# soon-yau/upgpt

Hardware: AMD Instinct MI355X
Metric: 256x256 images/sec, 50-step DDIM, bs=8/GPU; UNet MFMA util % (higher is better)
Workload: dtype f16; 1 GPU; BASELINE configs[1]: bs=8/GPU, 256x256 px (latent 4x32x32), 50-step DDIM eta=0, text-only cond [B,87,768], UNet(bbox.yaml) + VAE decode, EMA weights, no CFG; batch_per_gpu=8, ddim_steps=50, batches_in_flight_per_gpu=4, lane_hw_queues=measured, parallelism=replica-dp1, one all-gather of images per batch

## Files before the change

### include/upk.h

```cpp
#ifndef UPK_H_
#define UPK_H_

#include <stddef.h>
#include <stdint.h>

#ifdef __cplusplus
extern "C" {
#endif

#define UPK_VERSION 100

#define UPK_OK 0
#define UPK_EINVAL (-1)
#define UPK_ESHAPE (-2)
#define UPK_EWORKSPACE (-3)
#define UPK_EHIP (-4)
#define UPK_ENODEV (-5)

typedef struct upk_ctx upk_ctx;
typedef void* upk_stream;

int upk_version(void);
int upk_create(upk_ctx** out, int device);
int upk_destroy(upk_ctx* ctx);
const char* upk_last_error(upk_ctx* ctx);
int upk_set_workspace(upk_ctx* ctx, void* dptr, size_t bytes);
int upk_num_cus(upk_ctx* ctx);

int upk_pack_weight_f16(upk_ctx* ctx, const float* w_oihw, int cout, int cin, int kh, int kw,
                        const int32_t* row_map, int n_rows_packed, const int32_t* col_map,
                        int cin_packed, void* w_packed, upk_stream stream);
size_t upk_packed_weight_bytes(int n_rows_packed, int cin_packed, int kh, int kw);

#define UPK_F_SILU 0x1
#define UPK_F_GEGLU 0x2
#define UPK_F_OUT_F32 0x4
#define UPK_F_OUT_NCHW_F32 0x8
#define UPK_F_UPSAMPLE2X 0x10
#define UPK_F_PAD_ASYM 0x20
#define UPK_F_QUICKGELU 0x40

typedef struct upk_conv_desc {
  const void* x1;
  const void* x2;
  int32_t c1, c2;
  int32_t ld1, ld2;
  int32_t batch;
  int32_t in_h, in_w;
  int32_t ksize;
  int32_t stride;
  const void* w_packed;
  int32_t n_out;
  int32_t n_pad;
  const float* bias;
  const void* residual;
  int32_t ld_res;
  const float* rowvec;
  int32_t rv_batch_stride;
  int32_t rv_step_stride;
  const int32_t* step;
  void* y;
  int32_t ldy;
  void* vt;
  int32_t vt_from, vt_heads, vt_dhead, vt_ld, vt_tokens;
  int32_t flags;
  int32_t tune_cfg, tune_splitk;
  const float* ln_colsum;
  float ln_eps;
  int32_t ln_dim;
  float* gn_stats_ws;
  int32_t gn_groups;
  const void* x3;
  const void* x4;
  int32_t c3, c4;
  int32_t ld3, ld4;
  const float* gno_gamma;
  const float* gno_beta;
  void* gno_y;
  float gno_eps;
  int32_t gno_silu, gno_ld, gno_skip_y;
  float* ln_rows_out;
  const float* ln_rows_in;
  int32_t ln_rows_slots;
  const void* w_phase;
  int32_t gn_stats_cap;
  const void* pf_next;
  int64_t pf_bytes;
} upk_conv_desc;

int upk_conv2d_nhwc_f16(upk_ctx* ctx, const upk_conv_desc* d, upk_stream stream);

int upk_conv_gn_fused(upk_ctx* ctx, const upk_conv_desc* d, int* mode, int* nblk);
int upk_groupnorm_finalize_f32(upk_ctx* ctx, const float* partials, int nblk, int ld, int batch, int hw, int c,
                               int groups, float* ws, upk_stream stream);
int upk_conv_ln_rows(upk_ctx* ctx, const upk_conv_desc* d, int* slots);

typedef struct upk_mlp_desc {
  const void* x;
  int32_t ldx, m, c, inner;
  const void* w1;
  const float* b1;
  const float* u1;
  float ln_eps;
  int32_t ln_dim;
  const void* w2;
  const float* b2;
  int32_t n_out, n_pad;
  const void* residual;
  int32_t ld_res;
  void* y;
  int32_t ldy;
  float* gn_stats_ws;
  int32_t hw, rows_per_wg;
} upk_mlp_desc;
int upk_geglu_mlp_f16(upk_ctx* ctx, const upk_mlp_desc* d, upk_stream stream);
int upk_geglu_mlp_supported(upk_ctx* ctx, const upk_mlp_desc* d);

typedef struct upk_xblock_desc {
  const void* a1;
  int32_t lda, m, c, heads, d;
  const void* t0;
  int32_t ld_t0;
  const void* w_out1;
  const void* w_q;
  const void* w_out2;
  const float* vec;
  float ln_eps;
  int32_t ln_dim;
  const void* k_ctx;
  int32_t ldk, n_kv;
  const void* vt_ctx;
  int32_t vt_ld;
  float scale;
  void* y;
  int32_t ldy;
  int32_t hw, rows_per_wg;
} upk_xblock_desc;
int upk_cross_block_f16(upk_ctx* ctx, const upk_xblock_desc* d, upk_stream stream);
int upk_cross_block_supported(upk_ctx* ctx, const upk_xblock_desc* d);

typedef struct upk_hblock_desc {
  const void* x;
  int32_t ldx, m, c, heads, d;
  const void* w_in;
  const void* w_qkv;
  const float* vec;
  float ln_eps;
  int32_t ln_dim;
  void* t0;
  int32_t ld_t0;
  void* qk;
  int32_t ld_qk;
  void* vt;
  int32_t vt_ld;
  int32_t hw, rows_per_wg;
  const float* gn_part;
  const float* gn_gamma;
  const float* gn_beta;
  int32_t gn_nblk, gn_ld, gn_groups;
  float gn_eps;
} upk_hblock_desc;
int upk_head_block_f16(upk_ctx* ctx, const upk_hblock_desc* d, upk_stream stream);
int upk_head_block_supported(upk_ctx* ctx, const upk_hblock_desc* d);

int upk_gemm_f16(upk_ctx* ctx, const void* a, int lda, int m, int k, const void* w_packed,
                 int n_out, int n_pad, const float* bias, const void* residual, int ld_res,
                 void* y, int ldy, int flags, upk_stream stream);

int upk_conv_autotune(upk_ctx* ctx, const upk_conv_desc* d, upk_stream stream, int reps, int* best_cfg,
                      int* best_splitk, float* best_us, float* default_us);

int upk_conv_override(upk_ctx* ctx, int cfg, int splitk);
int upk_conv_num_configs(void);
const char* upk_conv_config_name(int cfg);

int upk_attention_f16(upk_ctx* ctx, const void* q, int ldq, long long q_batch_stride,
                      const void* k, int ldk, long long k_batch_stride, const void* vt, int vt_ld,
                      void* out, int ldo, long long o_batch_stride, int batch, int heads, int n_q,
                      int n_kv, int d, float scale, upk_stream stream);
// ... 180 lines not shown
```

### upgpt_amd/_lib.py

```python
import contextlib
import ctypes as C
import os
import threading

import torch
from ._check import require

_HERE = os.path.dirname(os.path.abspath(__file__))
LIB_PATH = os.environ.get("UPK_LIB") or os.path.join(_HERE, "libupk.so")

SYMBOLS = [
    "upk_version", "upk_create", "upk_destroy", "upk_last_error", "upk_set_workspace", "upk_num_cus",
    "upk_pack_weight_f16", "upk_packed_weight_bytes", "upk_conv2d_nhwc_f16", "upk_gemm_f16",
    "upk_conv_autotune", "upk_conv_override", "upk_conv_num_configs", "upk_conv_config_name", "upk_conv_gn_fused",
    "upk_conv_ln_rows",
    "upk_geglu_mlp_f16", "upk_geglu_mlp_supported", "upk_cross_block_f16", "upk_cross_block_supported", "upk_head_block_f16", "upk_head_block_supported",
    "upk_attention_f16", "upk_groupnorm_nhwc_f16", "upk_groupnorm_stats_nhwc_f16", "upk_groupnorm_chunks", "upk_groupnorm_apply_nhwc_f16", "upk_groupnorm_finalize_f32", "upk_groupnorm_ws_bytes",
    "upk_layernorm_f16", "upk_timestep_embed_f16",
    "upk_nchw_f32_to_nhwc_f16", "upk_nhwc_f16_to_nchw_f32", "upk_f32_to_f16", "upk_ddim_step_f32",
    "upk_ddim_step_cfg_f32", "upk_ddim_step_edit_f32", "upk_plms_step_f32", "upk_ddpm_step_f32", "upk_attention_causal_f16", "upk_attention_qproj_f16", "upk_embed_tokens_f16",
    "upk_attention_fewkeys_f16", "upk_gelu_f16",
    "upk_patchify_nchw_f32_f16", "upk_vit_assemble_f16", "upk_gather_rows_f16",
    "upk_image_finish_u8", "upk_resize_bilinear_u8", "upk_segm_boxes_u8", "upk_style_crops_u8",
    "upk_cond_bbox_u8", "upk_cond_gather_u8", "upk_cond_smpl_u8", "upk_clip_normalize_u8", "upk_ssim_ws_bytes", "upk_ssim_u8",
    "upk_lpips_input_f16", "upk_relu_pool_nhwc_f16", "upk_lpips_ws_bytes", "upk_lpips_layer_f16",
    "upk_conv2d_rect_f16", "upk_pool3_nhwc_f16", "upk_fid_input_f16", "upk_avgpool_global_f32",
    "upk_q_sample_f32", "upk_p_losses_ws_bytes", "upk_p_losses_f32",
    "upk_advance_step", "upk_step_autoadvance", "upk_kernel_launches", "upk_graph_begin", "upk_graph_end", "upk_graph_launch", "upk_graph_destroy",
    "upk_prof_enable", "upk_prof_collect",
    "upk_stream_create_cumask", "upk_stream_destroy", "upk_probe_placement", "upk_probe_clock",
]

F_SILU, F_GEGLU, F_OUT_F32, F_OUT_NCHW_F32, F_UPSAMPLE2X, F_PAD_ASYM = 0x1, 0x2, 0x4, 0x8, 0x10, 0x20
DDPM_X0, DDPM_CLIP = 0x1, 0x2
LAYOUT_NCHW, LAYOUT_NHWC = 0, 1
STYLE_FILL, STYLE_MASK = 0x1, 0x2
FINISH_SAMPLE, FINISH_INPUT, FINISH_DENORM = 0, 1, 2
F_QUICKGELU = 0x40
POOL_MAX, POOL_AVG = 0, 1
LOSS_L2, LOSS_L1 = 0, 1
NUM_CLASSES = 5
CLASS_NAMES = ["igemm", "attention", "groupnorm", "layernorm", "other"]

E_NAMES = {0: "UPK_OK", -1: "UPK_EINVAL", -2: "UPK_ESHAPE", -3: "UPK_EWORKSPACE", -4: "UPK_EHIP", -5: "UPK_ENODEV"}


class UpkError(RuntimeError):
    def __init__(self, code, msg):
        super().__init__("%s: %s" % (E_NAMES.get(code, str(code)), msg))
        self.code = code


class ConvDesc(C.Structure):
    _fields_ = [
        ("x1", C.c_void_p), ("x2", C.c_void_p),
        ("c1", C.c_int32), ("c2", C.c_int32), ("ld1", C.c_int32), ("ld2", C.c_int32),
        ("batch", C.c_int32), ("in_h", C.c_int32), ("in_w", C.c_int32),
        ("ksize", C.c_int32), ("stride", C.c_int32),
        ("w_packed", C.c_void_p), ("n_out", C.c_int32), ("n_pad", C.c_int32),
        ("bias", C.c_void_p), ("residual", C.c_void_p), ("ld_res", C.c_int32),
        ("rowvec", C.c_void_p), ("rv_batch_stride", C.c_int32), ("rv_step_stride", C.c_int32),
        ("step", C.c_void_p), ("y", C.c_void_p), ("ldy", C.c_int32),
        ("vt", C.c_void_p), ("vt_from", C.c_int32), ("vt_heads", C.c_int32), ("vt_dhead", C.c_int32),
        ("vt_ld", C.c_int32), ("vt_tokens", C.c_int32), ("flags", C.c_int32),
        ("tune_cfg", C.c_int32), ("tune_splitk", C.c_int32),
        ("ln_colsum", C.c_void_p), ("ln_eps", C.c_float), ("ln_dim", C.c_int32),
        ("gn_stats_ws", C.c_void_p), ("gn_groups", C.c_int32),
        ("x3", C.c_void_p), ("x4", C.c_void_p),
        ("c3", C.c_int32), ("c4", C.c_int32), ("ld3", C.c_int32), ("ld4", C.c_int32),
        ("gno_gamma", C.c_void_p), ("gno_beta", C.c_void_p), ("gno_y", C.c_void_p), ("gno_eps", C.c_float),
        ("gno_silu", C.c_int32), ("gno_ld", C.c_int32), ("gno_skip_y", C.c_int32),
        ("ln_rows_out", C.c_void_p), ("ln_rows_in", C.c_void_p), ("ln_rows_slots", C.c_int32),
        ("w_phase", C.c_void_p), ("gn_stats_cap", C.c_int32),
        ("pf_next", C.c_void_p), ("pf_bytes", C.c_int64),
    ]


class MlpDesc(C.Structure):
    _fields_ = [
        ("x", C.c_void_p), ("ldx", C.c_int32), ("m", C.c_int32), ("c", C.c_int32), ("inner", C.c_int32),
        ("w1", C.c_void_p), ("b1", C.c_void_p), ("u1", C.c_void_p), ("ln_eps", C.c_float), ("ln_dim", C.c_int32),
        ("w2", C.c_void_p), ("b2", C.c_void_p), ("n_out", C.c_int32), ("n_pad", C.c_int32),
        ("residual", C.c_void_p), ("ld_res", C.c_int32), ("y", C.c_void_p), ("ldy", C.c_int32),
        ("gn_stats_ws", C.c_void_p), ("hw", C.c_int32), ("rows_per_wg", C.c_int32),
    ]


class XblockDesc(C.Structure):
    _fields_ = [
        ("a1", C.c_void_p), ("lda", C.c_int32), ("m", C.c_int32), ("c", C.c_int32), ("heads", C.c_int32), ("d", C.c_int32),
        ("t0", C.c_void_p), ("ld_t0", C.c_int32),
        ("w_out1", C.c_void_p), ("w_q", C.c_void_p), ("w_out2", C.c_void_p), ("vec", C.c_void_p),
        ("ln_eps", C.c_float), ("ln_dim", C.c_int32),
        ("k_ctx", C.c_void_p), ("ldk", C.c_int32), ("n_kv", C.c_int32),
        ("vt_ctx", C.c_void_p), ("vt_ld", C.c_int32), ("scale", C.c_float),
        ("y", C.c_void_p), ("ldy", C.c_int32), ("hw", C.c_int32), ("rows_per_wg", C.c_int32),
    ]


class HblockDesc(C.Structure):
    _fields_ = [
        ("x", C.c_void_p), ("ldx", C.c_int32), ("m", C.c_int32), ("c", C.c_int32), ("heads", C.c_int32), ("d", C.c_int32),
        ("w_in", C.c_void_p), ("w_qkv", C.c_void_p), ("vec", C.c_void_p), ("ln_eps", C.c_float), ("ln_dim", C.c_int32),
        ("t0", C.c_void_p), ("ld_t0", C.c_int32), ("qk", C.c_void_p), ("ld_qk", C.c_int32),
        ("vt", C.c_void_p), ("vt_ld", C.c_int32), ("hw", C.c_int32), ("rows_per_wg", C.c_int32),
        ("gn_part", C.c_void_p), ("gn_gamma", C.c_void_p), ("gn_beta", C.c_void_p),
        ("gn_nblk", C.c_int32), ("gn_ld", C.c_int32), ("gn_groups", C.c_int32), ("gn_eps", C.c_float),
    ]


_lib = None
_lib_lock = threading.Lock()


def load_library(path=None):
    global _lib
    with _lib_lock:
        if _lib is not None and path is None:
            return _lib
        p = path or LIB_PATH
        if not os.path.exists(p):
            raise RuntimeError(
                "libupk.so not found at %s: build it with `python -m upgpt_amd.build` "
                "(hipcc --offload-arch=gfx950). There is no CPU fallback." % p)
        lib = C.CDLL(p)
        vp, i32, i64, f32 = C.c_void_p, C.c_int, C.c_longlong, C.c_float
        protos = {
            "upk_version": (C.c_int, []),
            "upk_create": (C.c_int, [C.POINTER(vp), i32]),
            "upk_destroy": (C.c_int, [vp]),
            "upk_last_error": (C.c_char_p, [vp]),
            "upk_set_workspace": (C.c_int, [vp, vp, C.c_size_t]),
            "upk_num_cus": (C.c_int, [vp]),
            "upk_pack_weight_f16": (C.c_int, [vp, vp, i32, i32, i32, i32, vp, i32, vp, i32, vp, vp]),
            "upk_packed_weight_bytes": (C.c_size_t, [i32, i32, i32, i32]),
            "upk_conv2d_nhwc_f16": (C.c_int, [vp, C.POINTER(ConvDesc), vp]),
            "upk_gemm_f16": (C.c_int, [vp, vp, i32, i32, i32, vp, i32, i32, vp, vp, i32, vp, i32, i32, vp]),
            "upk_conv_autotune": (C.c_int, [vp, C.POINTER(ConvDesc), vp, i32, C.POINTER(C.c_int), C.POINTER(C.c_int),
                                            C.POINTER(C.c_float), C.POINTER(C.c_float)]),
            "upk_conv_override": (C.c_int, [vp, i32, i32]),
            "upk_conv_num_configs": (C.c_int, []),
            "upk_conv_config_name": (C.c_char_p, [i32]),
            "upk_conv_ln_rows": (C.c_int, [vp, C.POINTER(ConvDesc), C.POINTER(C.c_int)]),
            "upk_geglu_mlp_f16": (C.c_int, [vp, C.POINTER(MlpDesc), vp]),
            "upk_geglu_mlp_supported": (C.c_int, [vp, C.POINTER(MlpDesc)]),
            "upk_cross_block_f16": (C.c_int, [vp, C.POINTER(XblockDesc), vp]),
            "upk_cross_block_supported": (C.c_int, [vp, C.POINTER(XblockDesc)]),
            "upk_head_block_f16": (C.c_int, [vp, C.POINTER(HblockDesc), vp]),
            "upk_head_block_supported": (C.c_int, [vp, C.POINTER(HblockDesc)]),
            "upk_attention_f16": (C.c_int, [vp, vp, i32, i64, vp, i32, i64, vp, i32, vp, i32, i64,
                                            i32, i32, i32, i32, i32, f32, vp]),
            "upk_attention_causal_f16": (C.c_int, [vp, vp, i32, i64, vp, i32, i64, vp, i32, vp, i32, i64,
                                                   i32, i32, i32, i32, f32, vp]),
            "upk_attention_qproj_f16": (C.c_int, [vp, vp, i32, i64, i32, i32, f32, vp, vp, vp, vp, i32, i64, vp, i32, vp,
                                                  i32, i64, i32, i32, i32, i32, i32, f32, vp]),
            "upk_attention_fewkeys_f16": (C.c_int, [vp, vp, i32, i64, vp, i32, i64, vp, i32, i64, vp, i32, i64,
                                                    i32, i32, i32, i32, i32, f32, vp]),
            "upk_gelu_f16": (C.c_int, [vp, vp, i32, i32, i32, vp]),
# ... 464 lines not shown
```

### upgpt_amd/csrc/mlp.hip

```cpp
#include "igemm_common.h"

namespace upkd {
namespace {

constexpr int ML_NW = 8;

struct MlpArgs {
  const f16* x;
  const f16* w1;
  const f16* w2;
  const f16* zero;
  const float* b1;
  const float* u1;
  const float* b2;
  const f16* res;
  f16* y;
  float* gn_cp;
  int ldx, ldr, ldy, M, nch1, n1, n2, n2pad, nh;
  int gn_nblk, gn_hw;
  float ln_inv_dim, ln_eps;
  unsigned long long* dbg;
};
#define ML_PIN(v) asm volatile("" ::"s"(v))

template <int MI, int PF>
__global__ __launch_bounds__(512) void mlp_kernel(const MlpArgs s) {
  constexpr int NW = ML_NW, NI = 2;
  constexpr int BM = MI * 16;
  constexpr int PW = NW * NI * 16;
  extern __shared__ __attribute__((aligned(16))) f16 smem[];
  ML_PIN(s.x); ML_PIN(s.w1); ML_PIN(s.w2); ML_PIN(s.zero); ML_PIN(s.b1); ML_PIN(s.u1); ML_PIN(s.b2); ML_PIN(s.res);
  ML_PIN(s.y); ML_PIN(s.gn_cp); ML_PIN(s.ldx); ML_PIN(s.ldr); ML_PIN(s.ldy); ML_PIN(s.M); ML_PIN(s.nch1); ML_PIN(s.n1);
  ML_PIN(s.n2); ML_PIN(s.n2pad); ML_PIN(s.nh);

  const int tid = threadIdx.x;
  const int lane = tid & 63;
  const int wave = __builtin_amdgcn_readfirstlane(tid >> 6);
  const int lg = lane >> 4, lc = lane & 15;
#ifdef UPK_TIMELINE
  const bool tl = s.dbg && (blockIdx.x == 0 || blockIdx.x == gridDim.x - 1) && (wave == 0 || wave == 4);
  unsigned long long* tlp = s.dbg + (blockIdx.x == 0 ? 0 : 64) + (wave == 0 ? 0 : 32);
#define STAMP(i) do { if (tl && lane == 0 && (i) < 32) tlp[i] = __builtin_readcyclecounter(); } while (0)
#else
#define STAMP(i) do { } while (0)
#endif
  STAMP(0);
  const int m0 = upk_xcd_tile(blockIdx.x, gridDim.x) * BM;
  const int nch1 = s.nch1, nh = s.nh, nch2 = nh + nch1;
  f16* const hT = smem;
  f16* const xT = smem + nh * BM * 32;
  float* const st = (float*)(smem + nch2 * BM * 32);
  float* const bl = st + BM * 2;

  {
    typedef __attribute__((address_space(3))) void* lds_ptr;
    typedef const __attribute__((address_space(1))) void* glb_ptr;
    const int r16 = lane >> 2;
    const int chd = (lane & 3) ^ ((-(lane >> 4)) & 3);
    const f16* zsrc = s.zero + (lane & 3) * 8;
    for (int idx = wave; idx < nch1 * MI; idx += NW) {
      const int kc = idx / MI, rg = idx - kc * MI;
      const int m = m0 + rg * 16 + r16;
      const f16* src = m < s.M ? s.x + (long)m * s.ldx + kc * 32 + chd * 8 : zsrc;
      __builtin_amdgcn_global_load_lds((glb_ptr)src, (lds_ptr)(xT + (kc * BM + rg * 16) * 32), 16, 0, 0);
    }
    const int nkb = s.n1 >> 8;
    for (int idx = wave; idx < 2 * nkb; idx += NW) {
      const float* src = (idx < nkb ? s.b1 + idx * 256 : s.u1 + (idx - nkb) * 256) + lane * 4;
      __builtin_amdgcn_global_load_lds((glb_ptr)src, (lds_ptr)(bl + idx * 256), 16, 0, 0);
    }
  }

  const int col1 = (wave >> 1) * 64 + (wave & 1) * 16;
  const int npass = (s.n1 + PW - 1) / PW;
  const int p1w = min(npass, (s.n1 - col1 + PW - 1) / PW);
  const int col2 = wave * 32;
  const bool act2 = col2 < s.n2pad;
  const unsigned ks1 = (unsigned)s.n1 * 64u, ks2 = (unsigned)s.n2pad * 64u;
  const unsigned loff = (unsigned)(lc * 32 + lg * 8) * 2u;
  unsigned voff1[PF], voff2[PF];
#pragma unroll
  for (int u = 0; u < PF; ++u) voff1[u] = loff + (unsigned)u * ks1, voff2[u] = loff + (unsigned)u * ks2;
  const char* wb1 = (const char*)s.w1;
  const char* wb2 = (const char*)s.w2 + (size_t)col2 * 64;
  auto base1 = [&](int p, int kc) -> const char* {
    return wb1 + (size_t)(((unsigned)kc * (unsigned)s.n1 + (unsigned)(col1 + p * PW)) * 64u);
  };
  f16x8 ring[PF][NI];
// ... 110 lines not shown
    STAMP(5 + 2 * p);
  }
  STAMP(20);
  __syncthreads();
  STAMP(21);

  if (!act2) return;
  f32x4 acc[MI][NI];
#pragma unroll
  for (int i = 0; i < MI; ++i)
#pragma unroll
    for (int j = 0; j < NI; ++j) acc[i][j] = (f32x4){0.f, 0.f, 0.f, 0.f};
#pragma unroll 1
  for (int kc0 = 0; kc0 < nch2; kc0 += PF) {
    const bool dead = kc0 + PF >= nch2;
    const char* sb0 = dead ? wb2 : wb2 + (size_t)((unsigned)(kc0 + PF) * ks2);
    const char* ldsA = hs + la + (unsigned)(kc0 * BM) * 64u;
#pragma unroll
    for (int u = 0; u < PF; ++u) {
      f16x8 fc[MI];
#pragma unroll
      for (int i = 0; i < MI; ++i) fc[i] = *(const f16x8*)(ldsA + (u * BM + i * 16) * 64);
#pragma unroll
      for (int i = 0; i < MI; ++i)
#pragma unroll
        for (int j = 0; j < NI; ++j)
          acc[i][j] = __builtin_amdgcn_mfma_f32_16x16x32_f16(ring[u][j], fc[i], acc[i][j], 0, 0, 0);
      const unsigned vo = dead ? loff : voff2[u];
      ring[u][0] = *(const f16x8*)(sb0 + vo);
      ring[u][1] = *(const f16x8*)(sb0 + (dead ? 0 : 1024) + vo);
      __builtin_amdgcn_sched_barrier(0);
    }
  }
  STAMP(22);
  f32x4 cs[NI], cq[NI];
#pragma unroll
  for (int j = 0; j < NI; ++j) cs[j] = cq[j] = (f32x4){0.f, 0.f, 0.f, 0.f};
#pragma unroll
  for (int i = 0; i < MI; ++i) {
    const int m = m0 + i * 16 + lc;
    const bool ok = m < s.M;
    f16* yrow = s.y + (unsigned)(ok ? m : 0) * (unsigned)s.ldy;
#pragma unroll
    for (int j = 0; j < NI; ++j) {
      const int n = col2 + j * 16 + lg * 4;
      const f32x4 v = acc[i][j] + b2v[j];
      f16x4 o;
#pragma unroll
      for (int k = 0; k < 4; ++k) o[k] = (f16)(v[k] + (float)rr[i][j][k]);
      if (ok && n < s.n2) *(f16x4*)(yrow + n) = o;
#pragma unroll
      for (int k = 0; k < 4; ++k) {
        const float f = ok ? (float)o[k] : 0.f;
        cs[j][k] += f;
        cq[j][k] += f * f;
      }
    }
  }
  if (s.gn_cp) {
    const int b = m0 / s.gn_hw;
    const int blk = (m0 - b * s.gn_hw) / BM;
    float* dst = s.gn_cp + (long)((b * s.gn_nblk + blk) * 2) * s.n2pad;
#pragma unroll
    for (int j = 0; j < NI; ++j) {
      const int n = col2 + j * 16 + lg * 4;
#pragma unroll
      for (int k = 0; k < 4; ++k) {
        cs[j][k] = Epi::row_sum16(cs[j][k]);
        cq[j][k] = Epi::row_sum16(cq[j][k]);
      }
      if (lc == 0 && n < s.n2pad) {
        *(f32x4*)(dst + n) = cs[j];
        *(f32x4*)(dst + s.n2pad + n) = cq[j];
      }
    }
  }
#ifdef UPK_TIMELINE
  asm volatile("s_waitcnt vmcnt(0)" ::: "memory");
  STAMP(23);
#endif
#undef STAMP
}

}
}

using namespace upkd;

extern "C" int upk_geglu_mlp_supported(upk_ctx* ctx, const upk_mlp_desc* d) {
  if (!ctx || !d) return 0;
  if (d->c <= 0 || (d->c & 31) || d->inner != 4 * d->c || (d->inner & 31)) return 0;
  const int nch1 = d->c / 32, nh = d->inner / 32;
  if (nch1 % 7 || (nch1 + nh) % 7) return 0;
  if (d->n_pad > ML_NW * 32 || (d->n_pad & 31)) return 0;
  if ((d->ldx & 7) || (d->ld_res & 3) || (d->ldy & 3) || (d->n_out & 3)) return 0;
  const int bm = d->rows_per_wg > 0 ? d->rows_per_wg : 64;
  if (bm != 32 && bm != 64) return 0;
  if ((2 * d->inner) & 255) return 0;
  if ((size_t)(nch1 + nh) * bm * 64 + (size_t)bm * 8 + (size_t)d->inner * 16 > 160 * 1024) return 0;
  if (d->gn_stats_ws && (d->hw <= 0 || d->hw % bm || d->hw / bm > UPK_GN_MAX_CHUNKS)) return 0;
  return 1;
}

extern "C" int upk_geglu_mlp_f16(upk_ctx* ctx, const upk_mlp_desc* d, upk_stream stream_) {
  if (!ctx || !d) return UPK_EINVAL;
  if (!d->x || !d->w1 || !d->w2 || !d->b1 || !d->u1 || !d->b2 || !d->residual || !d->y)
    return upk_fail(ctx, UPK_EINVAL, "geglu_mlp: null operand");
  if (!upk_geglu_mlp_supported(ctx, d))
    return upk_fail(ctx, UPK_ESHAPE, "geglu_mlp: shape outside the fused kernel's domain (c=%d inner=%d n_pad=%d)", d->c,
                    d->inner, d->n_pad);
  hipStream_t stream = (hipStream_t)stream_;
  MlpArgs s;
  memset(&s, 0, sizeof(s));
  s.x = (const f16*)d->x, s.w1 = (const f16*)d->w1, s.w2 = (const f16*)d->w2, s.zero = (const f16*)ctx->zero_page;
  s.b1 = d->b1, s.u1 = d->u1, s.b2 = d->b2, s.res = (const f16*)d->residual, s.y = (f16*)d->y;
  s.gn_cp = d->gn_stats_ws;
  s.ldx = d->ldx, s.ldr = d->ld_res, s.ldy = d->ldy, s.M = d->m;
  s.nch1 = d->c / 32, s.n1 = 2 * d->inner, s.n2 = d->n_out, s.n2pad = d->n_pad, s.nh = d->inner / 32;
  const int bm = d->rows_per_wg > 0 ? d->rows_per_wg : 64;
  s.gn_hw = d->hw > 0 ? d->hw : 1;
  s.gn_nblk = d->hw > 0 ? d->hw / bm : 1;
  s.ln_inv_dim = 1.0f / (float)(d->ln_dim > 0 ? d->ln_dim : d->c);
  s.ln_eps = d->ln_eps;
#ifdef UPK_TIMELINE
  s.dbg = getenv("UPK_MLP_TL") ? (unsigned long long*)((char*)ctx->ws + ctx->ws_bytes - 4096) : nullptr;
#endif
  const size_t lds = (size_t)(s.nch1 + s.nh) * bm * 64 + (size_t)bm * 8 + (size_t)s.n1 * 8;
  void (*fn)(const MlpArgs) = bm == 32 ? mlp_kernel<2, 7> : mlp_kernel<4, 7>;
  static unsigned long long attr32 = 0, attr64 = 0;
  if (int rc = upk_lds_attr_once(ctx, (const void*)fn, bm == 32 ? &attr32 : &attr64)) return rc;
  upk_prof_scope prof(ctx, UPK_CLS_IGEMM, stream);
  hipLaunchKernelGGL(fn, dim3((s.M + bm - 1) / bm), dim3(512), lds, stream, s);
  return upk_check_launch(ctx, "geglu_mlp");
}
```

### upgpt_amd/emitter.py

```python
import ctypes as C
import os

import torch

from . import _lib as L
from . import knobs as K
from ._check import require
from .packing import PW, Packer, _rup, head_pad
from .tuning import TUNE_CACHE, TUNE_CACHE_LANES


class Act:
    __slots__ = ("t", "B", "H", "W", "C", "gn_src", "ln_src")

    def __init__(self, t, B, H, W, C):
        self.t, self.B, self.H, self.W, self.C = t, B, H, W, C
        self.ln_src = None
        self.gn_src = None

    @property
    def ld(self):
        return self.t.shape[-1]

    @property
# ... 320 lines not shown
            if os.environ.get("UPGPT_GN_2SRC", "1") != "1":
                return None
            for sr in srcs:
                if isinstance(sr, Emitter.GnProvider):
                    continue
                key = self.convs[sr[1]][1]
                e = TUNE_CACHE.get(key) or TUNE_CACHE.get(key[:-3] if key.endswith("_gs") else key + "_gs")
                if e is None or (e[1] != 1 and not self._is_as(int(e[0]))):
                    return None
        armed = []
        for act in acts:
            if isinstance(act.gn_src, Emitter.GnProvider):
                armed.append((act.gn_src, act.gn_src.sws))
                continue
            d = act.gn_src[0]
            if not d.gn_stats_ws:
                ci = act.gn_src[1]
                cap = max(32, (act.H * act.W) // 64)
                sws = self.alloc(self.ctx.gn_stats_floats(act.B, d.n_pad, cap), dtype=torch.float32)
                d.gn_stats_ws, d.gn_groups, d.gn_stats_cap = sws.data_ptr(), 32, cap
                require(self.convs[ci][0] is d, "conv list out of sync with GroupNorm producers", RuntimeError)
                self.convs[ci] = (d, self.convs[ci][1] + "_gs")
                act.gn_src = (d, ci, sws)
            armed.append((d, act.gn_src[2]))
        return armed

    def groupnorm(self, P, x1, gamma, beta, eps, silu, ws, x2=None, sole=False):
        Cc = x1.C + (x2.C if x2 is not None else 0)
        y = Act(self.alloc(x1.M, Cc), x1.B, x1.H, x1.W, Cc)
        fn, h, chk = self.lib.upk_groupnorm_nhwc_f16, self.hctx, self._chk
        a = (x1.t.data_ptr(), x1.C, x1.ld, x2.t.data_ptr() if x2 is not None else None, x2.C if x2 is not None else 0,
             x2.ld if x2 is not None else 0, x1.B, x1.H * x1.W, 32, gamma.data_ptr(), beta.data_ptr(), float(eps),
             int(bool(silu)), y.t.data_ptr(), y.ld)
        armed = self._arm_gn_sources([x1] if x2 is None else [x1, x2])
        if armed is None:
            P.add(lambda s: chk(fn(h, *a, ws.data_ptr(), s)), x1, x2, gamma, beta, y, ws, cls="groupnorm",
                  label="gn M%d C%d silu%d 2pass" % (x1.M, Cc, int(bool(silu))))
        else:
            fused_fn, apply_fn = self.lib.upk_conv_gn_fused, self.lib.upk_groupnorm_apply_nhwc_f16
            fin_fn = self.lib.upk_groupnorm_finalize_f32
            mine = None
            if K.GN_REDUCE_APPLY and x2 is None and not isinstance(armed[0][0], Emitter.GnProvider) and not armed[0][0].gno_y:
                mine = armed[0][0]
                mine.gno_gamma, mine.gno_beta, mine.gno_eps = gamma.data_ptr(), beta.data_ptr(), float(eps)
                mine.gno_silu, mine.gno_y, mine.gno_ld, mine.gno_skip_y = int(bool(silu)), y.t.data_ptr(), y.ld, int(bool(sole))

            def run(s):
                info = []
                for d, sws in armed:
                    if isinstance(d, Emitter.GnProvider):
                        info.append((2, d.nblk, d.ld, sws.data_ptr()))
                        continue
                    mode, nblk = C.c_int(0), C.c_int(0)
                    chk(fused_fn(h, C.byref(d), C.byref(mode), C.byref(nblk)))
                    info.append((mode.value if mode.value != 3 or d is mine else 0, nblk.value, d.n_pad, sws.data_ptr()))
                if len(info) == 1 and info[0][0] == 3:
                    return
                if len(info) == 1 and info[0][0] == 2 and info[0][1] > 32:
                    m, nb, ld, p1 = info[0]
                    chk(fin_fn(h, p1, nb, ld, x1.B, x1.H * x1.W, x1.C, 32, ws.data_ptr(), s))
                    chk(apply_fn(h, *a, ws.data_ptr(), 1, 0, 0, None, 0, 0, s))
                    return
                if len(info) == 1 and info[0][0]:
                    m, nb, ld, p1 = info[0]
                    chk(apply_fn(h, *a, p1, m, nb, ld, None, 0, 0, s))
                elif len(info) == 2 and info[0][0] == 2 and info[1][0] == 2 and max(info[0][1], info[1][1]) <= 32:
                    chk(apply_fn(h, *a, info[0][3], 2, info[0][1], info[0][2], info[1][3], info[1][1], info[1][2], s))
                else:
                    chk(fn(h, *a, ws.data_ptr(), s))

            P.add(run, x1, x2, gamma, beta, y, ws, armed, cls="groupnorm",
                  label="gn M%d C%d silu%d" % (x1.M, Cc, int(bool(silu))))
        P.n_launch += 1
        return y

    def layernorm(self, P, x, gamma, beta, eps=1e-5):
        y = Act(self.alloc(x.M, x.C), x.B, x.H, x.W, x.C)
        fn, h, chk = self.lib.upk_layernorm_f16, self.hctx, self._chk
        a = (x.t.data_ptr(), x.ld, x.M, x.C, gamma.data_ptr(), beta.data_ptr(), float(eps), y.t.data_ptr(), y.ld)
        P.add(lambda s: chk(fn(h, *a, s)), x, gamma, beta, y, cls="layernorm", label="ln M%d C%d" % (x.M, x.C))
        return y

    def mlp_rows(self, M):
        if K.MLP_ROWS in (32, 64):
            return K.MLP_ROWS
        return 64 if M // 64 >= self.ctx.num_cus else 32

    def geglu_mlp(self, P, t2, x_in, pw1, pw2, gn_stats=True):
        if K.MLP_FUSE == "0" or t2.C != t2.ld:
            return None
        M, C_ = t2.M, t2.C
        if (K.MLP_FUSE == "auto" and L.concurrency() > 1 and os.environ.get("UPGPT_LANES_TUNING", "1") == "1"
                and M in TUNE_CACHE_LANES.meta.get("__unfuse_mlp_M__", ())):
            return None
        rows = self.mlp_rows(M)
        d = L.MlpDesc()
        d.x, d.ldx, d.m, d.c, d.inner = t2.t.data_ptr(), t2.ld, M, C_, pw1.n_out
        d.w1, d.b1, d.u1 = pw1.w.data_ptr(), pw1.bias.data_ptr(), pw1.ln_colsum.data_ptr()
        d.ln_eps, d.ln_dim = 1e-5, C_
        d.w2, d.b2, d.n_out, d.n_pad = pw2.w.data_ptr(), pw2.bias.data_ptr(), pw2.n_out, pw2.n_pad
        d.residual, d.ld_res = x_in.t.data_ptr(), x_in.ld
        hw = t2.H * t2.W
        d.hw, d.rows_per_wg = hw, rows
        if not self.lib.upk_geglu_mlp_supported(self.hctx, C.byref(d)):
            return None
        if K.MLP_FUSE == "auto" and (M + rows - 1) // rows < (self.ctx.num_cus * 3) // 4:
            return None
        out = Act(self.alloc(M, pw2.n_out), t2.B, t2.H, t2.W, pw2.n_out)
        d.y, d.ldy = out.t.data_ptr(), out.ld
        sws = None
        if gn_stats and hw % rows == 0 and hw // rows <= 32:
            sws = self.alloc(self.ctx.gn_stats_floats(t2.B, pw2.n_pad), dtype=torch.float32)
            d.gn_stats_ws = sws.data_ptr()
            out.gn_src = Emitter.GnProvider(sws, hw // rows, pw2.n_pad)
        fn, h, chk = self.lib.upk_geglu_mlp_f16, self.hctx, self._chk
        P.add(lambda s: chk(fn(h, C.byref(d), s)), d, t2, x_in, pw1, pw2, out, sws, cls="igemm_k1",
              label="mlp M%d C%d rows%d" % (M, C_, rows))
        P.igemm_flops += 2 * M * (2 * pw1.n_out * C_ + pw2.n_real * (pw1.n_out + C_))
        P.flops[-1] = 2 * M * (2 * pw1.n_out * C_ + pw2.n_real * (pw1.n_out + C_))
        return out

    def row_chain_rows(self, kind, M, default=32):
        forced = (K.HB_ROWS if kind == "hblock" else 0) or K.XB_ROWS
        if forced:
            return forced
        if L.concurrency() > 1 and os.environ.get("UPGPT_LANES_TUNING", "1") == "1":
            r = TUNE_CACHE_LANES.meta.get("__row_chain_rows__", {}).get(kind, {}).get(str(M))
            if r:
                return int(r)
        return default

    def head_block_ok(self, x, t, heads, dp, qk, vt_ld):
        if K.HBLOCK == "0" or (t + ".hblock.vec") not in self.pk.w or x.C % 32:
            return False
        rows = self.row_chain_rows("hblock", x.M)
        d = L.HblockDesc()
        d.ldx, d.m, d.c, d.heads, d.d = x.C, x.M, x.C, heads, dp
        d.ld_t0, d.ld_qk, d.vt_ld, d.hw, d.rows_per_wg = x.C, qk.ld, vt_ld, x.H * x.W, rows
        if not self.lib.upk_head_block_supported(self.hctx, C.byref(d)):
            return False
        return K.HBLOCK == "1" or x.M // min(rows, 32) >= self.ctx.num_cus

    def head_block(self, P, x, n, t, heads, dp, qk, vt, vt_ld, gn):
        w = self.pk.w
        vec = w[t + ".hblock.vec"]
        gamma, beta, eps, ws = gn
        M, C_ = x.M, x.C
        hw = x.H * x.W
        rows = self.row_chain_rows("hblock", M)
        pi, qkv = w[n + ".proj_in"], w[t + ".attn1.qkv_ln"]
        armed = self._arm_gn_sources([x]) if K.HBLOCK_GN else None
        if armed is None:
            xn = self.groupnorm(P, x, gamma, beta, eps, False, ws)
        else:
            xn = Act(self.alloc(M, C_), x.B, x.H, x.W, C_)
        d = L.HblockDesc()
        d.x, d.ldx, d.m, d.c, d.heads, d.d = xn.t.data_ptr(), xn.ld, M, C_, heads, dp
        d.w_in, d.w_qkv, d.vec = pi.w.data_ptr(), qkv.w.data_ptr(), vec.data_ptr()
        d.ln_eps, d.ln_dim = 1e-5, C_
        d.qk, d.ld_qk, d.vt, d.vt_ld = qk.t.data_ptr(), qk.ld, vt.data_ptr(), vt_ld
        d.hw, d.rows_per_wg = hw, rows
        require(self.lib.upk_head_block_supported(self.hctx, C.byref(d)), "head_block: unsupported shape", RuntimeError)
        t0 = Act(self.alloc(M, C_), x.B, x.H, x.W, C_)
        d.t0, d.ld_t0 = t0.t.data_ptr(), t0.ld
        fn, h, chk = self.lib.upk_head_block_f16, self.hctx, self._chk
        label = "hblock M%d C%d d%d rows%d" % (M, C_, dp, rows)
        if armed is None:
            P.add(lambda s: chk(fn(h, C.byref(d), s)), d, xn, pi, qkv, vec, t0, qk, vt, cls="igemm_k1", label=label)
        else:
            fused_fn, apply_fn = self.lib.upk_conv_gn_fused, self.lib.upk_groupnorm_apply_nhwc_f16
            fin_fn, gn_fn = self.lib.upk_groupnorm_finalize_f32, self.lib.upk_groupnorm_nhwc_f16
            a = (x.t.data_ptr(), x.C, x.ld, None, 0, 0, x.B, hw, 32, gamma.data_ptr(), beta.data_ptr(), float(eps), 0,
                 xn.t.data_ptr(), xn.ld)
            src, sws = armed[0]
            mine = None
            if K.GN_REDUCE_APPLY and not isinstance(src, Emitter.GnProvider) and not src.gno_y:
                mine = src
                mine.gno_gamma, mine.gno_beta, mine.gno_eps = gamma.data_ptr(), beta.data_ptr(), float(eps)
                mine.gno_silu, mine.gno_y, mine.gno_ld, mine.gno_skip_y = 0, xn.t.data_ptr(), xn.ld, 0

            def run(s):
                if isinstance(src, Emitter.GnProvider):
                    mode, nb, ld = 2, src.nblk, src.ld
                else:
                    m_, n_ = C.c_int(0), C.c_int(0)
                    chk(fused_fn(h, C.byref(src), C.byref(m_), C.byref(n_)))
                    mode, nb, ld = (m_.value if m_.value != 3 or src is mine else 0), n_.value, src.n_pad
                if mode == 3:
                    d.x, d.ldx, d.gn_part = xn.t.data_ptr(), xn.ld, None
                    chk(fn(h, C.byref(d), s))
                    return
                if mode == 2 and nb <= 32:
                    d.x, d.ldx = x.t.data_ptr(), x.ld
                    d.gn_part, d.gn_gamma, d.gn_beta = sws.data_ptr(), gamma.data_ptr(), beta.data_ptr()
                    d.gn_nblk, d.gn_ld, d.gn_groups, d.gn_eps = nb, ld, 32, float(eps)
                    chk(fn(h, C.byref(d), s))
                    return
                if mode == 2:
                    chk(fin_fn(h, sws.data_ptr(), nb, ld, x.B, hw, x.C, 32, ws.data_ptr(), s))
                    chk(apply_fn(h, *a, ws.data_ptr(), 1, 0, 0, None, 0, 0, s))
                elif mode:
                    chk(apply_fn(h, *a, sws.data_ptr(), mode, nb, ld, None, 0, 0, s))
                else:
                    chk(gn_fn(h, *a, ws.data_ptr(), s))
                d.x, d.ldx, d.gn_part = xn.t.data_ptr(), xn.ld, None
                chk(fn(h, C.byref(d), s))

            P.add(run, d, x, xn, gamma, beta, ws, armed, pi, qkv, vec, t0, qk, vt, cls="igemm_k1", label=label + " gn")
        fl = 2 * M * (pi.k_real * pi.n_real + qkv.k_real * qkv.n_real)
        P.igemm_flops += fl
# ... 44 lines not shown
```

### upgpt_amd/knobs.py

```python
import os

VAE_GN_BYPRODUCT = os.environ.get("UPGPT_VAE_GN_BYPRODUCT", "0")
VAE_GN_MINM = int(os.environ.get("UPGPT_VAE_GN_MINM", "131072"))


def vae_gn_byproduct(M):
    return VAE_GN_BYPRODUCT == "1" or (VAE_GN_BYPRODUCT == "auto" and M >= VAE_GN_MINM)
UPS_PHASES = os.environ.get("UPGPT_UPS_PHASES", "1") == "1"
LN_ROWS = os.environ.get("UPGPT_LN_ROWS", "1") == "1"
QPROJ_FUSE = os.environ.get("UPGPT_QPROJ_FUSE", "1") == "1"
GN_REDUCE_APPLY = os.environ.get("UPGPT_GN_REDUCE_APPLY", "1") == "1"
MLP_FUSE = os.environ.get("UPGPT_MLP_FUSE", "auto")
MLP_ROWS = int(os.environ.get("UPGPT_MLP_ROWS", "0"))
XBLOCK = os.environ.get("UPGPT_XBLOCK", "auto")
XB_ROWS = int(os.environ.get("UPGPT_XB_ROWS", "0"))
HB_ROWS = int(os.environ.get("UPGPT_HB_ROWS", "0"))
HBLOCK = os.environ.get("UPGPT_HBLOCK", "auto")
HBLOCK_GN = os.environ.get("UPGPT_HBLOCK_GN", "1") == "1"
WEIGHT_PREFETCH = os.environ.get("UPGPT_WEIGHT_PREFETCH", "auto")
WEIGHT_PREFETCH_AHEAD = int(os.environ.get("UPGPT_WEIGHT_PREFETCH_AHEAD", "1"))
WEIGHT_PREFETCH_MAX = int(os.environ.get("UPGPT_WEIGHT_PREFETCH_MAX", str(32 << 20)))
LN_LAUNCH_US = 5.0
```

Before: 98.72 images/s.

## Add streaming GEGLU MLP kernel that slices the hidden tile through LDS

New measurement: 100.6 images/s, median of 6. +1.9%, better.

```diff
diff --git a/include/upk.h b/include/upk.h
--- a/include/upk.h
+++ b/include/upk.h
@@ -95,6 +95,7 @@
                                int groups, float* ws, upk_stream stream);
 int upk_conv_ln_rows(upk_ctx* ctx, const upk_conv_desc* d, int* slots);
 
+#define UPK_MLP_STREAM 0x1000
 typedef struct upk_mlp_desc {
   const void* x;
   int32_t ldx, m, c, inner;
diff --git a/upgpt_amd/_lib.py b/upgpt_amd/_lib.py
--- a/upgpt_amd/_lib.py
+++ b/upgpt_amd/_lib.py
@@ -74,6 +74,9 @@
         ("w_phase", C.c_void_p), ("gn_stats_cap", C.c_int32),
         ("pf_next", C.c_void_p), ("pf_bytes", C.c_int64),
     ]
+
+
+MLP_STREAM = 0x1000
 
 
 class MlpDesc(C.Structure):
diff --git a/upgpt_amd/csrc/mlp.hip b/upgpt_amd/csrc/mlp.hip
--- a/upgpt_amd/csrc/mlp.hip
+++ b/upgpt_amd/csrc/mlp.hip
@@ -4,6 +4,9 @@
 namespace {
 
 constexpr int ML_NW = 8;
+#ifndef UPK_MLP_SLICES
+#define UPK_MLP_SLICES 2
+#endif
 
 struct MlpArgs {
   const f16* x;
@@ -280,10 +283,279 @@
 #undef STAMP
 }
 
+template <int I>
+struct ml_ic {
+  static constexpr int value = I;
+};
+template <int B, int E, class F>
+__device__ __forceinline__ void ml_static_for(F&& f) {
+  if constexpr (B < E) {
+    f(ml_ic<B>{});
+    ml_static_for<B + 1, E>(f);
+  }
+}
+
+template <int MI, int RD>
+__global__ __launch_bounds__(512) void mlp_stream_kernel(const MlpArgs s) {
+  constexpr int NW = ML_NW, NI = 2;
+  constexpr int BM = MI * 16;
+  constexpr int PW = NW * NI * 16;
+  constexpr int NK1 = 7;
+  constexpr int NS = PW / 64;
+  constexpr int S = NK1 + NS;
+  constexpr int NSL = UPK_MLP_SLICES;
+  static_assert(RD >= 1 && RD <= NK1, "the first RD steps of a pass are w1 chunks (t2 chunks behind the last pass)");
+  extern __shared__ __attribute__((aligned(16))) f16 smem[];
+  ML_PIN(s.x); ML_PIN(s.w1); ML_PIN(s.w2); ML_PIN(s.zero); ML_PIN(s.b1); ML_PIN(s.u1); ML_PIN(s.b2); ML_PIN(s.res);
+  ML_PIN(s.y); ML_PIN(s.gn_cp); ML_PIN(s.ldx); ML_PIN(s.ldr); ML_PIN(s.ldy); ML_PIN(s.M); ML_PIN(s.nch1); ML_PIN(s.n1);
+  ML_PIN(s.n2); ML_PIN(s.n2pad); ML_PIN(s.nh);
+
+  const int tid = threadIdx.x;
+  const int lane = tid & 63;
+  const int wave = __builtin_amdgcn_readfirstlane(tid >> 6);
+  const int lg = lane >> 4, lc = lane & 15;
+  const int m0 = upk_xcd_tile(blockIdx.x, gridDim.x) * BM;
+  const int nh = s.nh;
+  f16* const xT = smem;
+  f16* const hS = smem + NK1 * BM * 32;
+  float* const st = (float*)(smem + (NK1 + NSL * NS) * BM * 32);
+  float* const bl = st + BM * 2;
+
+  {
+    typedef __attribute__((address_space(3))) void* lds_ptr;
+    typedef const __attribute__((address_space(1))) void* glb_ptr;
+    const int r16 = lane >> 2;
+    const int chd = (lane & 3) ^ ((-(lane >> 4)) & 3);
+    const f16* zsrc = s.zero + (lane & 3) * 8;
+    for (int idx = wave; idx < NK1 * MI; idx += NW) {
+      const int kc = idx / MI, rg = idx - kc * MI;
+      const int m = m0 + rg * 16 + r16;
+      const f16* src = m < s.M ? s.x + (long)m * s.ldx + kc * 32 + chd * 8 : zsrc;
+      __builtin_amdgcn_global_load_lds((glb_ptr)src, (lds_ptr)(xT + (kc * BM + rg * 16) * 32), 16, 0, 0);
+    }
+    const int nkb = s.n1 >> 8;
+    for (int idx = wave; idx < 2 * nkb; idx += NW) {
+      const float* src = (idx < nkb ? s.b1 + idx * 256 : s.u1 + (idx - nkb) * 256) + lane * 4;
+      __builtin_amdgcn_global_load_lds((glb_ptr)src, (lds_ptr)(bl + idx * 256), 16, 0, 0);
+    }
+  }
+
+  const int col1 = (wave >> 1) * 64 + (wave & 1) * 16;
+  const int npass = s.n1 / PW;
+  const int col2 = wave * 32;
+  const bool act2 = col2 < s.n2pad;
+  const unsigned ks1 = (unsigned)s.n1 * 64u, ks2 = act2 ? (unsigned)s.n2pad * 64u : 0u;
+  const unsigned loff = (unsigned)(lc * 32 + lg * 8) * 2u;
+  const char* wb1 = (const char*)s.w1 + (size_t)col1 * 64;
+  const char* wb2 = (const char*)s.w2 + (size_t)(act2 ? col2 : 0) * 64;
+  const char* const wt2 = wb2 + (size_t)((unsigned)nh * ks2);
+  f16x8 ring[RD][NI];
+#pragma unroll
+  for (int u = 0; u < RD; ++u) {
+    ring[u][0] = *(const f16x8*)(wb1 + (unsigned)u * ks1 + loff);
+    ring[u][1] = *(const f16x8*)(wb1 + (unsigned)u * ks1 + 2048 + loff);
+  }
+  __syncthreads();
+
+  {
+    constexpr int LPR = 512 / BM;
+    const int row = tid / LPR, part = tid - row * LPR;
+    float s1 = 0.f, s2 = 0.f;
+    const f16x2 one2 = {(f16)1.f, (f16)1.f};
+    for (int q = part; q < NK1 * 4; q += LPR) {
+      const f16x8 v = *(const f16x8*)(xT + ((q >> 2) * BM + row) * 32 + (q & 3) * 8);
+#pragma unroll
+      for (int h = 0; h < 4; ++h) {
+        const f16x2 xx = {v[2 * h], v[2 * h + 1]};
+        s1 = __builtin_amdgcn_fdot2(xx, one2, s1, false);
+        s2 = __builtin_amdgcn_fdot2(xx, xx, s2, false);
+      }
+    }
+#pragma unroll
+    for (int o = 1; o < LPR; o <<= 1) {
+      s1 += __shfl_xor(s1, o);
+      s2 += __shfl_xor(s2, o);
+    }
+    if (part == 0) {
+      const float mu = s1 * s.ln_inv_dim;
+      st[2 * row] = mu;
+      st[2 * row + 1] = rsqrtf(fmaxf(s2 * s.ln_inv_dim - mu * mu, 0.f) + s.ln_eps);
+    }
+  }
+  __syncthreads();
+
+  const unsigned la = (unsigned)(lc * 32 + lds_swz(lc, lg) * 8) * 2u;
+  const char* const xs = (const char*)xT + la;
+  f32x4 acc[MI][NI];
+#pragma unroll
+  for (int i = 0; i < MI; ++i)
+#pragma unroll
+    for (int j = 0; j < NI; ++j) acc[i][j] = (f32x4){0.f, 0.f, 0.f, 0.f};
+
+#pragma unroll 1
+  for (int p = 0; p < npass; ++p) {
+    const bool last = p + 1 >= npass;
+    const char* const g1 = wb1 + (size_t)((unsigned)(p * PW) * 64u);
+    const char* const g2 = wb2 + (size_t)((unsigned)(p * NS) * ks2);
+    const char* const nx = last ? wt2 : g1 + PW * 64;
+    const unsigned ksn = last ? ks2 : ks1, fn = last ? 1024u : 2048u;
+    f16* const hT = hS + (p % NSL) * (NS * BM * 32);
+    auto refill = [&](auto tc) {
+      constexpr int t = decltype(tc)::value, q = t + RD, sl = t % RD;
+      if constexpr (q < NK1) {
+        ring[sl][0] = *(const f16x8*)(g1 + (unsigned)q * ks1 + loff);
+        ring[sl][1] = *(const f16x8*)(g1 + (unsigned)q * ks1 + 2048 + loff);
+      } else if constexpr (q < S) {
+        ring[sl][0] = *(const f16x8*)(g2 + (unsigned)(q - NK1) * ks2 + loff);
+        ring[sl][1] = *(const f16x8*)(g2 + (unsigned)(q - NK1) * ks2 + 1024 + loff);
+      } else {
+        ring[sl][0] = *(const f16x8*)(nx + (unsigned)sl * ksn + loff);
+        ring[sl][1] = *(const f16x8*)(nx + (unsigned)sl * ksn + fn + loff);
+      }
+    };
+    f32x4 ag[MI][NI];
+#pragma unroll
+    for (int i = 0; i < MI; ++i)
+#pragma unroll
+      for (int j = 0; j < NI; ++j) ag[i][j] = (f32x4){0.f, 0.f, 0.f, 0.f};
+    ml_static_for<0, NK1>([&](auto tc) {
+      constexpr int t = decltype(tc)::value;
+      f16x8 fc[MI];
+#pragma unroll
+      for (int i = 0; i < MI; ++i) fc[i] = *(const f16x8*)(xs + (t * BM + i * 16) * 64);
+#pragma unroll
+      for (int i = 0; i < MI; ++i)
+#pragma unroll
+        for (int j = 0; j < NI; ++j)
+          ag[i][j] = __builtin_amdgcn_mfma_f32_16x16x32_f16(ring[t % RD][j], fc[i], ag[i][j], 0, 0, 0);
+      refill(tc);
+      __builtin_amdgcn_sched_barrier(0);
+    });
+    {
+      const int n = col1 + p * PW + lg * 4;
+      const f32x4 bv0 = *(const f32x4*)(bl + n), bv1 = *(const f32x4*)(bl + n + 32);
+      const f32x4 lu0 = *(const f32x4*)(bl + s.n1 + n), lu1 = *(const f32x4*)(bl + s.n1 + n + 32);
+      const int oc = n & 31;
+      const int hk = wave >> 1, hq = oc >> 3, hh = oc & 7;
+#pragma unroll
+      for (int i = 0; i < MI; ++i) {
+        const f32x2 mr = *(const f32x2*)(st + 2 * (i * 16 + lc));
+        const f32x4 v = (ag[i][0] - mr[0] * lu0) * mr[1] + bv0;
+        const f32x4 g = (ag[i][1] - mr[0] * lu1) * mr[1] + bv1;
+        f16x4 o;
+#pragma unroll
+        for (int k = 0; k < 4; ++k) o[k] = (f16)upk_geglu_mul(v[k], g[k]);
+        const int row = i * 16 + lc;
+        *(f16x4*)(hT + (hk * BM + row) * 32 + lds_swz(lc, hq) * 8 + hh) = o;
+      }
+    }
+    __syncthreads();
+    const char* const hs = (const char*)hT + la;
+    ml_static_for<NK1, S>([&](auto tc) {
+      constexpr int t = decltype(tc)::value;
+      f16x8 fc[MI];
+#pragma unroll
+      for (int i = 0; i < MI; ++i) fc[i] = *(const f16x8*)(hs + ((t - NK1) * BM + i * 16) * 64);
+#pragma unroll
+      for (int i = 0; i < MI; ++i)
+#pragma unroll
+        for (int j = 0; j < NI; ++j)
+          acc[i][j] = __builtin_amdgcn_mfma_f32_16x16x32_f16(ring[t % RD][j], fc[i], acc[i][j], 0, 0, 0);
+      refill(tc);
+      __builtin_amdgcn_sched_barrier(0);
+    });
+    if constexpr (NSL == 1) __syncthreads();
+  }
+
+  if (!act2) return;
+  f32x4 b2v[NI];
+  f16x4 rr[MI][NI];
+#pragma unroll
+  for (int j = 0; j < NI; ++j) {
+    const int n = col2 + j * 16 + lg * 4;
+    b2v[j] = *(const f32x4*)(s.b2 + n);
+#pragma unroll
+    for (int i = 0; i < MI; ++i) {
+      const unsigned m = (unsigned)min(m0 + i * 16 + lc, s.M - 1);
+      rr[i][j] = *(const f16x4*)(s.res + m * (unsigned)s.ldr + (unsigned)(n < s.n2 ? n : 0));
+    }
+  }
+  __builtin_amdgcn_sched_barrier(0);
+  ml_static_for<0, NK1>([&](auto tc) {
+    constexpr int t = decltype(tc)::value;
+    f16x8 fc[MI];
+#pragma unroll
+    for (int i = 0; i < MI; ++i) fc[i] = *(const f16x8*)(xs + (t * BM + i * 16) * 64);
+#pragma unroll
+    for (int i = 0; i < MI; ++i)
+#pragma unroll
+      for (int j = 0; j < NI; ++j)
+        acc[i][j] = __builtin_amdgcn_mfma_f32_16x16x32_f16(ring[t % RD][j], fc[i], acc[i][j], 0, 0, 0);
+    if constexpr (t + RD < NK1) {
+      ring[t % RD][0] = *(const f16x8*)(wt2 + (unsigned)(t + RD) * ks2 + loff);
+      ring[t % RD][1] = *(const f16x8*)(wt2 + (unsigned)(t + RD) * ks2 + 1024 + loff);
+    }
+    __builtin_amdgcn_sched_barrier(0);
+  });
+  f32x4 cs[NI], cq[NI];
+#pragma unroll
+  for (int j = 0; j < NI; ++j) cs[j] = cq[j] = (f32x4){0.f, 0.f, 0.f, 0.f};
+#pragma unroll
+  for (int i = 0; i < MI; ++i) {
+    const int m = m0 + i * 16 + lc;
+    const bool ok = m < s.M;
+    f16* yrow = s.y + (unsigned)(ok ? m : 0) * (unsigned)s.ldy;
+#pragma unroll
+    for (int j = 0; j < NI; ++j) {
+      const int n = col2 + j * 16 + lg * 4;
+      const f32x4 v = acc[i][j] + b2v[j];
+      f16x4 o;
+#pragma unroll
+      for (int k = 0; k < 4; ++k) o[k] = (f16)(v[k] + (float)rr[i][j][k]);
+      if (ok && n < s.n2) *(f16x4*)(yrow + n) = o;
+#pragma unroll
+      for (int k = 0; k < 4; ++k) {
+        const float f = ok ? (float)o[k] : 0.f;
+        cs[j][k] += f;
+        cq[j][k] += f * f;
+      }
+    }
+  }
+  if (s.gn_cp) {
+    const int b = m0 / s.gn_hw;
+    const int blk = (m0 - b * s.gn_hw) / BM;
+    float* dst = s.gn_cp + (long)((b * s.gn_nblk + blk) * 2) * s.n2pad;
+#pragma unroll
+    for (int j = 0; j < NI; ++j) {
+      const int n = col2 + j * 16 + lg * 4;
+#pragma unroll
+      for (int k = 0; k < 4; ++k) {
+        cs[j][k] = Epi::row_sum16(cs[j][k]);
+        cq[j][k] = Epi::row_sum16(cq[j][k]);
+      }
+      if (lc == 0) {
+        *(f32x4*)(dst + n) = cs[j];
+        *(f32x4*)(dst + s.n2pad + n) = cq[j];
+      }
+    }
+  }
+}
+
 }
 }
 
 using namespace upkd;
+
+static int mlp_form(const upk_mlp_desc* d, int* stream) {
+  const int raw = d->rows_per_wg > 0 ? d->rows_per_wg : 64;
+  const int bm = (raw & ~UPK_MLP_STREAM) ? (raw & ~UPK_MLP_STREAM) : 64;
+  *stream = (raw & UPK_MLP_STREAM) != 0 || bm == 128;
+  return bm;
+}
+
+static size_t mlp_lds_bytes(int nch1, int nh, int n1, int bm, int stream) {
+  return (size_t)(stream ? nch1 + 4 * UPK_MLP_SLICES : nch1 + nh) * bm * 64 + (size_t)bm * 8 + (size_t)n1 * 8;
+}
 
 extern "C" int upk_geglu_mlp_supported(upk_ctx* ctx, const upk_mlp_desc* d) {
   if (!ctx || !d) return 0;
@@ -292,10 +564,12 @@
   if (nch1 % 7 || (nch1 + nh) % 7) return 0;
   if (d->n_pad > ML_NW * 32 || (d->n_pad & 31)) return 0;
   if ((d->ldx & 7) || (d->ld_res & 3) || (d->ldy & 3) || (d->n_out & 3)) return 0;
-  const int bm = d->rows_per_wg > 0 ? d->rows_per_wg : 64;
-  if (bm != 32 && bm != 64) return 0;
+  int stream;
+  const int bm = mlp_form(d, &stream);
+  if (stream ? (bm != 64 && bm != 128) : (bm != 32 && bm != 64)) return 0;
   if ((2 * d->inner) & 255) return 0;
-  if ((size_t)(nch1 + nh) * bm * 64 + (size_t)bm * 8 + (size_t)d->inner * 16 > 160 * 1024) return 0;
+  if (mlp_lds_bytes(nch1, nh, 2 * d->inner, bm, stream) > 160 * 1024) return 0;
+  if (stream && nch1 != 7) return 0;
   if (d->gn_stats_ws && (d->hw <= 0 || d->hw % bm || d->hw / bm > UPK_GN_MAX_CHUNKS)) return 0;
   return 1;
 }
@@ -315,7 +589,8 @@
   s.gn_cp = d->gn_stats_ws;
   s.ldx = d->ldx, s.ldr = d->ld_res, s.ldy = d->ldy, s.M = d->m;
   s.nch1 = d->c / 32, s.n1 = 2 * d->inner, s.n2 = d->n_out, s.n2pad = d->n_pad, s.nh = d->inner / 32;
-  const int bm = d->rows_per_wg > 0 ? d->rows_per_wg : 64;
+  int strm;
+  const int bm = mlp_form(d, &strm);
   s.gn_hw = d->hw > 0 ? d->hw : 1;
   s.gn_nblk = d->hw > 0 ? d->hw / bm : 1;
   s.ln_inv_dim = 1.0f / (float)(d->ln_dim > 0 ? d->ln_dim : d->c);
@@ -323,10 +598,11 @@
 #ifdef UPK_TIMELINE
   s.dbg = getenv("UPK_MLP_TL") ? (unsigned long long*)((char*)ctx->ws + ctx->ws_bytes - 4096) : nullptr;
 #endif
-  const size_t lds = (size_t)(s.nch1 + s.nh) * bm * 64 + (size_t)bm * 8 + (size_t)s.n1 * 8;
-  void (*fn)(const MlpArgs) = bm == 32 ? mlp_kernel<2, 7> : mlp_kernel<4, 7>;
-  static unsigned long long attr32 = 0, attr64 = 0;
-  if (int rc = upk_lds_attr_once(ctx, (const void*)fn, bm == 32 ? &attr32 : &attr64)) return rc;
+  const size_t lds = mlp_lds_bytes(s.nch1, s.nh, s.n1, bm, strm);
+  void (*fn)(const MlpArgs) = strm ? (bm == 64 ? mlp_stream_kernel<4, 7> : mlp_stream_kernel<8, 4>)
+                                     : (bm == 32 ? mlp_kernel<2, 7> : mlp_kernel<4, 7>);
+  static unsigned long long attr[4] = {0, 0, 0, 0};
+  if (int rc = upk_lds_attr_once(ctx, (const void*)fn, &attr[strm * 2 + (bm > (strm ? 64 : 32))])) return rc;
   upk_prof_scope prof(ctx, UPK_CLS_IGEMM, stream);
   hipLaunchKernelGGL(fn, dim3((s.M + bm - 1) / bm), dim3(512), lds, stream, s);
   return upk_check_launch(ctx, "geglu_mlp");
diff --git a/upgpt_amd/emitter.py b/upgpt_amd/emitter.py
--- a/upgpt_amd/emitter.py
+++ b/upgpt_amd/emitter.py
@@ -426,7 +426,7 @@
         return y
 
     def mlp_rows(self, M):
-        if K.MLP_ROWS in (32, 64):
+        if K.MLP_ROWS in (32, 64, 128):
             return K.MLP_ROWS
         return 64 if M // 64 >= self.ctx.num_cus else 32
 
@@ -434,10 +434,12 @@
         if K.MLP_FUSE == "0" or t2.C != t2.ld:
             return None
         M, C_ = t2.M, t2.C
-        if (K.MLP_FUSE == "auto" and L.concurrency() > 1 and os.environ.get("UPGPT_LANES_TUNING", "1") == "1"
+        rows = self.row_chain_rows("mlp", M, 0)
+        if (not rows and K.MLP_FUSE == "auto" and L.concurrency() > 1 and os.environ.get("UPGPT_LANES_TUNING", "1") == "1"
                 and M in TUNE_CACHE_LANES.meta.get("__unfuse_mlp_M__", ())):
             return None
-        rows = self.mlp_rows(M)
+        rows = rows or self.mlp_rows(M)
+        stream = rows == 128 or (rows == 64 and K.MLP_STREAM)
         d = L.MlpDesc()
         d.x, d.ldx, d.m, d.c, d.inner = t2.t.data_ptr(), t2.ld, M, C_, pw1.n_out
         d.w1, d.b1, d.u1 = pw1.w.data_ptr(), pw1.bias.data_ptr(), pw1.ln_colsum.data_ptr()
@@ -445,10 +447,10 @@
         d.w2, d.b2, d.n_out, d.n_pad = pw2.w.data_ptr(), pw2.bias.data_ptr(), pw2.n_out, pw2.n_pad
         d.residual, d.ld_res = x_in.t.data_ptr(), x_in.ld
         hw = t2.H * t2.W
-        d.hw, d.rows_per_wg = hw, rows
+        d.hw, d.rows_per_wg = hw, rows | (L.MLP_STREAM if stream else 0)
         if not self.lib.upk_geglu_mlp_supported(self.hctx, C.byref(d)):
             return None
-        if K.MLP_FUSE == "auto" and (M + rows - 1) // rows < (self.ctx.num_cus * 3) // 4:
+        if K.MLP_FUSE == "auto" and (M + min(rows, 32) - 1) // min(rows, 32) < (self.ctx.num_cus * 3) // 4:
             return None
         out = Act(self.alloc(M, pw2.n_out), t2.B, t2.H, t2.W, pw2.n_out)
         d.y, d.ldy = out.t.data_ptr(), out.ld
@@ -459,17 +461,19 @@
             out.gn_src = Emitter.GnProvider(sws, hw // rows, pw2.n_pad)
         fn, h, chk = self.lib.upk_geglu_mlp_f16, self.hctx, self._chk
         P.add(lambda s: chk(fn(h, C.byref(d), s)), d, t2, x_in, pw1, pw2, out, sws, cls="igemm_k1",
-              label="mlp M%d C%d rows%d" % (M, C_, rows))
+              label="mlp M%d C%d rows%d%s" % (M, C_, rows, "s" if stream else ""))
         P.igemm_flops += 2 * M * (2 * pw1.n_out * C_ + pw2.n_real * (pw1.n_out + C_))
         P.flops[-1] = 2 * M * (2 * pw1.n_out * C_ + pw2.n_real * (pw1.n_out + C_))
         return out
 
     def row_chain_rows(self, kind, M, default=32):
-        forced = (K.HB_ROWS if kind == "hblock" else 0) or K.XB_ROWS
+        forced = K.MLP_ROWS if kind == "mlp" else (K.HB_ROWS if kind == "hblock" else 0) or K.XB_ROWS
         if forced:
             return forced
         if L.concurrency() > 1 and os.environ.get("UPGPT_LANES_TUNING", "1") == "1":
-            r = TUNE_CACHE_LANES.meta.get("__row_chain_rows__", {}).get(kind, {}).get(str(M))
+            tab = (TUNE_CACHE_LANES.meta.get("__mlp_rows__", {}) if kind == "mlp"
+                   else TUNE_CACHE_LANES.meta.get("__row_chain_rows__", {}).get(kind, {}))
+            r = tab.get(str(M))
             if r:
                 return int(r)
         return default
diff --git a/upgpt_amd/knobs.py b/upgpt_amd/knobs.py
--- a/upgpt_amd/knobs.py
+++ b/upgpt_amd/knobs.py
@@ -12,6 +12,7 @@
 GN_REDUCE_APPLY = os.environ.get("UPGPT_GN_REDUCE_APPLY", "1") == "1"
 MLP_FUSE = os.environ.get("UPGPT_MLP_FUSE", "auto")
 MLP_ROWS = int(os.environ.get("UPGPT_MLP_ROWS", "0"))
+MLP_STREAM = os.environ.get("UPGPT_MLP_STREAM", "0") == "1"
 XBLOCK = os.environ.get("UPGPT_XBLOCK", "auto")
 XB_ROWS = int(os.environ.get("UPGPT_XB_ROWS", "0"))
 HB_ROWS = int(os.environ.get("UPGPT_HB_ROWS", "0"))
```
